# CYF2000127/MolNexTR

Hardware: AMD Instinct MI355X
Metric: molecules/sec (384x384, bs32 per GPU), full predict hot path (higher is better)
Workload: dtype fp16x3

## Files before the change

### molnextr_amd/csrc/engine.hip

```cpp
#include "../../include/molnextr_hip.h"

#include <hip/hip_runtime.h>

#include <time.h>
#include <cmath>
#include <cstdint>
#include <cstdio>
#include <cstring>
#include <map>
#include <memory>
#include <string>
#include <tuple>
#include <unordered_map>
#include <vector>

#include "dec_types.h"
#include "kernels.h"
#include "kvq.h"

using namespace mnx;

namespace {

thread_local std::string g_create_error;

struct W16 {
    void* p = nullptr;
    size_t lo = 0;
    float oscale = 1.f;
};
struct BlockW {
    float *ln1_g, *ln1_b, *table, *qkv_b, *proj_b, *ln2_g, *ln2_b, *fc1_b, *fc2_b;
    W16 qkv_w, proj_w, fc1_w, fc2_w;
};
struct StageW {
    std::vector<BlockW> blocks;
    float *m_g = nullptr, *m_b = nullptr;
    W16 m_w;
    int C = 0, heads = 0;
};
enum { SPL_QKV = 1, SPL_ATTN = 2, SPL_PROJ = 4, SPL_FC1 = 8, SPL_FC2 = 16, SPL_MERGE = 32, SPL_ALL = 63 };
struct GraphKey {
    int slots, rows, trace, forced, tile;
    bool operator<(const GraphKey& o) const {
        return std::tie(slots, rows, trace, forced, tile) < std::tie(o.slots, o.rows, o.trace, o.forced, o.tile);
    }
};

}

#ifndef MNX_PLANE_SKEW
#define MNX_PLANE_SKEW 4352
#endif
static constexpr size_t PLANE_SKEW = MNX_PLANE_SKEW;

struct mnx_engine {
    mnx_config cfg;
    int device = 0;
    std::string err;
    std::vector<void*> allocs;
    size_t bytes = 0;
    float *pe_wt = nullptr, *pe_b = nullptr, *pe_g = nullptr, *pe_beta = nullptr, *fn_g = nullptr, *fn_b = nullptr;
    std::vector<StageW> stages;
    float *xa = nullptr, *xb = nullptr;
    void *xn16 = nullptr, *qkv16 = nullptr, *attn16 = nullptr, *h16 = nullptr;
    size_t xn_lo = 0, qkv_lo = 0, attn_lo = 0, h_lo = 0;
    int dt = 0;
    int split_mask = SPL_ALL;
    int two_mask[4] = {0, 0, 0, 0};
    int two_first[4] = {0, 0, 0, 0}, two_last[4] = {1 << 30, 1 << 30, 1 << 30, 1 << 30};
    int* enc_flag = nullptr;
    float* zero_bias = nullptr;
    int zero_bias_n = 0;
    int tap_item = -1;
    float* tap_dst = nullptr;
    DecWeights dw{};
    DecBuffers db{};
    float* out_trace = nullptr;
    int* forced_ids = nullptr;
    BeamBuffers beam{};
    int* prep_bbox = nullptr;
    int* prep_bbox_batch = nullptr;
    float* beam_hidden = nullptr;
    int* host_flag = nullptr;
    std::map<GraphKey, hipGraphExec_t> graphs;
    hipStream_t enc_stream = nullptr;
    float* feat_ring[2] = {nullptr, nullptr};
    hipEvent_t ev_enc_done[2] = {nullptr, nullptr}, ev_feat_free[2] = {nullptr, nullptr}, ev_poll[2] = {nullptr, nullptr};
    int* slot_lists = nullptr;
    int* rowc_seq = nullptr;
    TokenClasses* tc_dev = nullptr;
    bool have_tc = false;
    int n_chunk_bufs = 0;
    bool use_graph = true;
    int dec_tile = -1, dec_tile_ff = 4, dec_fused_max = 128;
    int dec_mid_max = 0;
    hipStream_t own_stream = nullptr;
    bool profiling = false;
    int prof_stride = 1;
    int prof_calls = 0;
    int prof_groups = 0;
    int prof_max_groups = 4;
    struct Ev { hipEvent_t a, b; double work; int kind; };
    std::vector<Ev> ev_pool;
    size_t ev_used = 0;
};

namespace {

#define HIPCHK(h, expr)                                                                                   \
    do {                                                                                                  \
        hipError_t e_ = (expr);                                                                           \
        if (e_ != hipSuccess) {                                                                           \
            (h)->err = std::string(#expr) + ": " + hipGetErrorString(e_);                                 \
            return MNX_ERR_HIP;                                                                           \
        }                                                                                                 \
    } while (0)

#define MNXCHK(expr)                                                                                      \
    do {                                                                                                  \
        const int rc_ = (expr);                                                                           \
        if (rc_ != MNX_OK) return rc_;                                                                    \
    } while (0)

struct Packer {
    mnx_engine* h;
    std::unordered_map<std::string, const mnx_weight_desc*> by_name;
    std::vector<std::string> problems;
    float* staging = nullptr;
    size_t staging_elems = 0;

    const mnx_weight_desc* find(const std::string& name, std::initializer_list<int64_t> shape) {
        auto it = by_name.find(name);
        if (it == by_name.end()) {
            problems.push_back("missing " + name);
            return nullptr;
        }
        const mnx_weight_desc* d = it->second;
        bool ok = d->ndim == (int)shape.size() && d->data != nullptr;
        int i = 0;
        for (int64_t s : shape) ok = ok && d->shape[i++] == s;
        if (!ok) {
            std::string got = "[";
            for (int k = 0; k < d->ndim; ++k) got += std::to_string(d->shape[k]) + (k + 1 < d->ndim ? "," : "");
            problems.push_back("shape " + name + ": got " + got + "]");
            return nullptr;
        }
        return d;
    }
    void* dalloc(size_t bytes) {
        void* p = nullptr;
        if (hipMalloc(&p, bytes ? bytes : 16) != hipSuccess) {
            problems.push_back("hipMalloc failed for " + std::to_string(bytes) + " bytes");
            return nullptr;
        }
        h->allocs.push_back(p);
        h->bytes += bytes;
        return p;
    }
    float* up32(const float* host, size_t n) {
        float* p = (float*)dalloc(n * sizeof(float));
        if (p && hipMemcpy(p, host, n * sizeof(float), hipMemcpyHostToDevice) != hipSuccess)
            problems.push_back("hipMemcpy H2D failed");
        return p;
    }
    float* f32(const std::string& name, std::initializer_list<int64_t> shape) {
        const mnx_weight_desc* d = find(name, shape);
        if (!d) return nullptr;
        size_t n = 1;
// ... 494 lines not shown
    h->err = "encoder features are not finite (an activation left the fp16 range of compute_dtype FP16 / FP16X3, or the "
             "input holds NaN / Inf): use MNX_DTYPE_BF16X3 or MNX_DTYPE_FP32 for this checkpoint";
    return MNX_ERR_RANGE;
}

static int encode_impl(mnx_engine* h, const char* name, const void* images, int fmt, int32_t B, float* features_out,
                       void* stream) {
    if (!h) return MNX_ERR_INVALID_ARG;
    if (!images || !features_out || B < 1) { h->err = std::string(name) + ": null/empty argument"; return MNX_ERR_INVALID_ARG; }
    if (fmt == MNX_IMG_GRAY8 && ((uintptr_t)images & 3)) { h->err = std::string(name) + ": gray must be 4-byte aligned"; return MNX_ERR_INVALID_ARG; }
    if (B > h->cfg.max_batch) { h->err = std::string(name) + ": B exceeds max_batch"; return MNX_ERR_CAPACITY; }
    hipStream_t s = (hipStream_t)stream;
    const mnx_config& c = h->cfg;
    const int dt = h->dt;
    HIPCHK(h, hipSetDevice(h->device));
    int Hh = c.img_size / c.patch, Ww = Hh, C = c.embed_dim;
    float* cur = h->xa;
    float* other = h->xb;
    int item = 0;
    auto tap = [&](size_t elems) -> hipError_t {
        hipError_t e = hipSuccess;
        if (h->tap_item == item && h->tap_dst)
            e = hipMemcpyAsync(h->tap_dst, cur, elems * sizeof(float), hipMemcpyDeviceToDevice, s);
        ++item;
        return e;
    };
    const bool bracket = h->profiling && (h->prof_calls++ % h->prof_stride) == 0 && h->prof_groups < h->prof_max_groups;
    if (bracket) ++h->prof_groups;
    auto timed = [&](int kind, double work, auto&& launch) -> hipError_t {
        if (!bracket) return launch();
        if (h->ev_used == h->ev_pool.size()) {
            mnx_engine::Ev ev{};
            hipError_t e1 = hipEventCreate(&ev.a), e2 = hipEventCreate(&ev.b);
            if (e1 != hipSuccess || e2 != hipSuccess) return e1 != hipSuccess ? e1 : e2;
            h->ev_pool.push_back(ev);
        }
        mnx_engine::Ev& ev = h->ev_pool[h->ev_used++];
        ev.work = work; ev.kind = kind;
        hipError_t e0 = hipEventRecord(ev.a, s);
        if (e0 != hipSuccess) return e0;
        e0 = launch();
        if (e0 != hipSuccess) return e0;
        return hipEventRecord(ev.b, s);
    };
    const double es = (double)dt_size(dt);
    const bool split = dt_split(dt);
    int stage_now = 0, block_now = 0;
    auto terms_of = [&](int cls) {
        if (!(h->split_mask & cls)) return 1;
        const bool in_range = block_now >= h->two_first[stage_now] && block_now <= h->two_last[stage_now];
        return (in_range && (h->two_mask[stage_now] & cls)) ? 2 : 3;
    };
    auto planes_for = [&](int consumer_cls) { return split && terms_of(consumer_cls) == 2 ? 1 : 2; };
    auto gemm = [&](int epi, const void* A, size_t a_lo, const W16& Wt, void* Cc, size_t c_lo, const float* bias,
                    const float* resid, int M, int N, int K, int cls, int c_planes = 2) -> hipError_t {
        SplitArgs sp;
        sp.a_lo = a_lo; sp.w_lo = Wt.lo; sp.c_lo = c_lo; sp.oscale = Wt.oscale;
        sp.terms = terms_of(cls);
        sp.c_planes = c_planes;
        return timed((cls != SPL_MERGE && std::min(N, K) >= 512) ? 4 : 0, 2.0 * (double)M * (double)N * (double)K,
                     [&]() { return launch_gemm16(dt, epi, A, Wt.p, Cc, bias, resid, M, N, K, s, split ? &sp : nullptr); });
    };
    auto ln = [&](const float* x, const float* g, const float* b, void* y16, float* y32, int M, int Cc, int planes = 2) -> hipError_t {
        return timed(1, (double)M * Cc * (4.0 + (y16 ? es * planes / 2 : 0.0) + (y32 ? 4.0 : 0.0)),
                     [&]() { return launch_layernorm16(dt, x, g, b, y16, y32, M, Cc, 1e-5f, s, h->xn_lo, y32 ? h->enc_flag : nullptr, planes); });
    };
    if (fmt == MNX_IMG_GRAY8)
        HIPCHK(h, timed(3, (double)B * ((double)c.img_size * c.img_size + (double)Hh * Ww * C * 4.0), [&]() {
            return launch_patch_embed_gray8((const uint8_t*)images, h->pe_wt, h->pe_b, h->pe_g, h->pe_beta, cur, B, c.img_size, C, s);
        }));
    else
        HIPCHK(h, timed(3, (double)B * (3.0 * c.img_size * c.img_size + (double)Hh * Ww * C) * 4.0, [&]() {
            return launch_patch_embed((const float*)images, h->pe_wt, h->pe_b, h->pe_g, h->pe_beta, cur, B, c.img_size, C, s);
        }));
    HIPCHK(h, tap((size_t)B * Hh * Ww * C));
    for (int si = 0; si < c.n_stages; ++si) {
        StageW& st = h->stages[si];
        stage_now = si;
        const int M = B * Hh * Ww;
        for (size_t bi = 0; bi < st.blocks.size(); ++bi) {
            const BlockW& w = st.blocks[bi];
            block_now = (int)bi;
            const int shift = (bi % 2 == 0) ? 0 : c.window / 2;
            HIPCHK(h, ln(cur, w.ln1_g, w.ln1_b, h->xn16, nullptr, M, C, planes_for(SPL_QKV)));
            HIPCHK(h, gemm(EPI_BIAS_16, h->xn16, h->xn_lo, w.qkv_w, h->qkv16, h->qkv_lo, w.qkv_b, nullptr, M, 3 * C, C, SPL_QKV));
            HIPCHK(h, timed(2, (double)M * C * 4.0 * es, [&]() {
                return launch_window_attn(dt, h->qkv16, w.table, h->attn16, B, Hh, Ww, C, st.heads, shift, s, h->qkv_lo,
                                          h->attn_lo, (h->split_mask & SPL_ATTN) ? 3 : 1);
            }));
            HIPCHK(h, gemm(EPI_RESID_F32, h->attn16, h->attn_lo, w.proj_w, cur, 0, w.proj_b, cur, M, C, C, SPL_PROJ));
            HIPCHK(h, ln(cur, w.ln2_g, w.ln2_b, h->xn16, nullptr, M, C, planes_for(SPL_FC1)));
            HIPCHK(h, gemm(EPI_GELU_16, h->xn16, h->xn_lo, w.fc1_w, h->h16, h->h_lo, w.fc1_b, nullptr, M, 4 * C, C, SPL_FC1, planes_for(SPL_FC2)));
            HIPCHK(h, gemm(EPI_RESID_F32, h->h16, h->h_lo, w.fc2_w, cur, 0, w.fc2_b, cur, M, C, 4 * C, SPL_FC2));
            HIPCHK(h, tap((size_t)M * C));
        }
        if (si + 1 < c.n_stages) {
            block_now = (int)st.blocks.size() - 1;
            HIPCHK(h, launch_merge_ln16(dt, cur, st.m_g, st.m_b, h->xn16, B, Hh, Ww, C, 1e-5f, s, h->xn_lo, planes_for(SPL_MERGE)));
            HIPCHK(h, gemm(EPI_BIAS_F32, h->xn16, h->xn_lo, st.m_w, other, 0, h->zero_bias, nullptr, M / 4, 2 * C, 4 * C, SPL_MERGE));
            std::swap(cur, other);
            Hh /= 2; Ww /= 2; C *= 2;
            HIPCHK(h, tap((size_t)B * Hh * Ww * C));
        }
    }
    HIPCHK(h, ln(cur, h->fn_g, h->fn_b, nullptr, features_out, B * Hh * Ww, C));
    return MNX_OK;
}

int mnx_encode(mnx_engine* h, const float* images, int32_t B, float* features_out, void* stream) {
    return encode_impl(h, "mnx_encode", images, MNX_IMG_F32, B, features_out, stream);
}

int mnx_encode_gray8(mnx_engine* h, const uint8_t* gray, int32_t B, float* features_out, void* stream) {
    return encode_impl(h, "mnx_encode_gray8", gray, MNX_IMG_GRAY8, B, features_out, stream);
}

}

namespace {

int caller_stream(mnx_engine* h, void* stream, hipStream_t* s) {
    HIPCHK(h, hipSetDevice(h->device));
    *s = (hipStream_t)stream;
    if (!*s) {
        if (!h->own_stream) HIPCHK(h, hipStreamCreate(&h->own_stream));
        *s = h->own_stream;
    }
    return MNX_OK;
}

template <typename T>
int lazy_alloc(mnx_engine* h, T** p, size_t bytes) {
    if (*p) return MNX_OK;
    HIPCHK(h, hipMalloc((void**)p, bytes));
    h->allocs.push_back(*p);
    h->bytes += bytes;
    return MNX_OK;
}

int project_memory(mnx_engine* h, const float* feats, int n, int blk0, hipStream_t s) {
    const mnx_config& c = h->cfg;
    const int S = h->db.S, D = c.dec_dim;
    char* memkv = h->db.mem_kv + (size_t)blk0 * c.dec_layers * 2 * c.dec_heads * kvq_block_bytes(h->db.Sq);
    HIPCHK(h, launch_sgemm_tn(feats, h->dw.w_enc, h->dw.b_enc, h->db.memory, n * S, D, h->dw.enc_dim, s));
    HIPCHK(h, launch_sgemm_tn(h->db.memory, h->dw.w_memkv, h->dw.b_memkv, h->db.mem_kv32, n * S, c.dec_layers * 2 * D, D, s, S));
    HIPCHK(h, kvq_pack_enqueue(h->db.mem_kv32, memkv, n * c.dec_layers * 2 * c.dec_heads, S, h->db.Sq, s));
    return MNX_OK;
}

struct FeatRing {
    mnx_engine* h;
    const void* images;
    int fmt;
    int n_img, ref_batch, n_chunks, grp;
    int first[2] = {-1, -1}, count[2] = {0, 0};
    bool used[2] = {false, false};
    int next_enc = 0;

    int refill() {
        const size_t img_bytes = (size_t)h->cfg.img_size * h->cfg.img_size * (fmt == MNX_IMG_GRAY8 ? 1 : 3 * sizeof(float));
        for (int i = 0; i < 2; ++i) {
            if (first[i] >= 0 || next_enc >= n_chunks) continue;
            const int cnt = std::min(grp, n_chunks - next_enc);
            const int f = next_enc * ref_batch, n = std::min(cnt * ref_batch, n_img - f);
            if (used[i]) HIPCHK(h, hipStreamWaitEvent(h->enc_stream, h->ev_feat_free[i], 0));
            MNXCHK(encode_impl(h, fmt == MNX_IMG_GRAY8 ? "mnx_encode_gray8" : "mnx_encode", (const char*)images + (size_t)f * img_bytes,
                               fmt, n, h->feat_ring[i], h->enc_stream));
            HIPCHK(h, hipEventRecord(h->ev_enc_done[i], h->enc_stream));
            first[i] = next_enc;
            count[i] = cnt;
            next_enc += cnt;
        }
        return MNX_OK;
    }
    int find(int k) const {
        for (int i = 0; i < 2; ++i)
            if (first[i] >= 0 && k >= first[i] && k < first[i] + count[i]) return i;
        return -1;
    }
    int end(int i) const { return first[i] + count[i]; }
    const float* feats(int i, int k) const {
        return h->feat_ring[i] + (size_t)(k - first[i]) * ref_batch * h->db.S * h->dw.enc_dim;
    }
    int release(int i, hipStream_t s) {
        HIPCHK(h, hipEventRecord(h->ev_feat_free[i], s));
        used[i] = true;
        first[i] = -1;
        return MNX_OK;
    }
};

struct DrainGuard {
    mnx_engine* h;
    hipStream_t s;
    ~DrainGuard() { (void)hipStreamSynchronize(h->enc_stream); (void)hipStreamSynchronize(s); }
};

int tick_tile(const mnx_engine* h, int rows) {
    const mnx_config& c = h->cfg;
    if (c.dec_ff != 1024 || c.dec_heads != 8 || c.dec_dim != 256 || c.max_len + 1 > 512 || h->db.S > 160) return 0;
    if (h->dec_tile == 0 || rows % 16 || rows > h->db.fpart_rows) return 0;
    if (rows > h->dec_fused_max) {
        if (rows > h->dec_mid_max) return 0;
        return 2000 + 100 * 4 + 16;
    }
    const int r = h->dec_tile > 0 ? h->dec_tile : (rows <= 64 ? 2 : 4);
    return 100 * r + h->dec_tile_ff;
}

hipError_t enqueue_tick(mnx_engine* h, int slots, int rows, float* trace, int trace_rows, hipStream_t s, const int* forced) {
    return dec_enqueue_tick(h->dw, h->db, slots, rows, trace, trace_rows, s, nullptr, forced, tick_tile(h, rows));
}

template <typename F>
int capture_graph(mnx_engine* h, const char* what, hipStream_t s, F&& enqueue, hipGraphExec_t* out) {
    *out = nullptr;
    HIPCHK(h, hipStreamBeginCapture(s, hipStreamCaptureModeThreadLocal));
    hipGraph_t g = nullptr;
    hipError_t e = enqueue();
    const hipError_t e2 = hipStreamEndCapture(s, &g);
    if (e == hipSuccess) e = e2;
    const char* step = "capture";
    if (e == hipSuccess) {
        step = "instantiate";
        e = hipGraphInstantiate(out, g, nullptr, nullptr, 0);
    }
    if (g) hipGraphDestroy(g);
    if (e != hipSuccess) {
        *out = nullptr;
        h->err = std::string(what) + " " + step + " failed: " + hipGetErrorString(e);
        return MNX_ERR_HIP;
    }
    return MNX_OK;
}

int get_tick_graph(mnx_engine* h, int slots, int rows, float* trace, int trace_rows, hipStream_t s, hipGraphExec_t* out,
                   const int* forced = nullptr) {
    *out = nullptr;
    if (!h->use_graph) return MNX_OK;
    const GraphKey key{slots, rows, trace ? trace_rows : 0, forced ? trace_rows : 0, tick_tile(h, rows)};
    auto it = h->graphs.find(key);
    if (it != h->graphs.end()) { *out = it->second; return MNX_OK; }
    MNXCHK(capture_graph(h, "decode tick", s, [&]() { return enqueue_tick(h, slots, rows, trace, trace_rows, s, forced); }, out));
    h->graphs[key] = *out;
    return MNX_OK;
}

template <typename F>
int run_steps(mnx_engine* h, hipGraphExec_t exec, F&& enqueue, int slots, int max_len, hipStream_t s) {
    for (int t = 0; t < max_len; t += 8) {
        for (int i = 0; i < std::min(8, max_len - t); ++i) HIPCHK(h, exec ? hipGraphLaunch(exec, s) : enqueue());
        HIPCHK(h, dec_enqueue_status(h->db, slots, s));
        HIPCHK(h, hipMemcpyAsync(h->host_flag, &h->db.st->n_active, sizeof(int), hipMemcpyDeviceToHost, s));
        HIPCHK(h, hipStreamSynchronize(s));
        if (*h->host_flag == 0) break;
    }
    return MNX_OK;
}

int decode_greedy_impl(mnx_engine* h, const float* features, int32_t B, const int32_t* chunk_id, int32_t max_len,
                       int32_t stop_on_eos, const int32_t* forced_ids, int32_t* tokens, int32_t* lengths, float* token_logp,
                       float* hidden, float* logits_trace, void* stream) {
    if (!h) return MNX_ERR_INVALID_ARG;
    if (!features || !tokens || !lengths || B < 1) { h->err = "mnx_decode_greedy: null/empty argument"; return MNX_ERR_INVALID_ARG; }
    if (B > ROW_TILE || max_len < 1 || max_len > h->cfg.max_len) {
        h->err = "mnx_decode_greedy: B must be <= 32 and max_len <= cfg.max_len";
        return MNX_ERR_CAPACITY;
    }
    const mnx_config& c = h->cfg;
    hipStream_t s;
    MNXCHK(caller_stream(h, stream, &s));
    MNXCHK(project_memory(h, features, B, 0, s));
    HIPCHK(h, dec_enqueue_reset(h->db, s));
    HIPCHK(h, dec_enqueue_admit_rows(h->db, chunk_id, B, max_len, stop_on_eos, s));
    float* trace = nullptr;
    if (logits_trace) {
        MNXCHK(lazy_alloc(h, &h->out_trace, (size_t)c.max_len * ROW_TILE * c.vocab * 4));
        trace = h->out_trace;
    }
    const int* forced = nullptr;
    if (forced_ids) {
        MNXCHK(lazy_alloc(h, &h->forced_ids, (size_t)ROW_TILE * c.max_len * 4));
        HIPCHK(h, hipMemcpy2DAsync(h->forced_ids, (size_t)h->db.T * 4, forced_ids, (size_t)max_len * 4, (size_t)max_len * 4, B,
                                   hipMemcpyDeviceToDevice, s));
        forced = h->forced_ids;
    }
    hipGraphExec_t exec = nullptr;
    MNXCHK(get_tick_graph(h, ROW_TILE, ROW_TILE, trace, B, s, &exec, forced));
    MNXCHK(run_steps(h, exec, [&]() { return enqueue_tick(h, ROW_TILE, ROW_TILE, trace, B, s, forced); }, ROW_TILE, max_len, s));
    HIPCHK(h, gather_enqueue(h->db, nullptr, B, max_len, tokens, lengths, token_logp, hidden, s));
    if (logits_trace) HIPCHK(h, hipMemcpyAsync(logits_trace, trace, (size_t)max_len * B * c.vocab * 4, hipMemcpyDeviceToDevice, s));
    HIPCHK(h, hipStreamSynchronize(s));
    return MNX_OK;
}

int decode_beam_groups(mnx_engine* h, const float* const* feats, int G, int ref_batch, int n_total, int beam, int n_best,
                       int max_len, int32_t* tokens, int32_t* lengths, float* scores, float* hidden, hipStream_t s) {
    const int D = h->cfg.dec_dim, T = h->db.T, B = n_total;
    BeamBuffers& bm = h->beam;
    constexpr int POOL = ROW_TILE * MAX_BEAM;
    const int pool_stride = std::min(MAX_BEAM, POOL / B);
    if (pool_stride < n_best) { h->err = "beam search: n_best x images exceeds the hypothesis pool (256)"; return MNX_ERR_CAPACITY; }
    MNXCHK(lazy_alloc(h, &bm.bs, sizeof(BeamState)));
    MNXCHK(lazy_alloc(h, &bm.blp, (size_t)MAX_BEAM_IMGS * MAX_BEAM * BEAM_LP_STRIDE * 4));
    MNXCHK(lazy_alloc(h, &bm.anc, (size_t)MAX_BEAM_IMGS * MAX_BEAM * (T + 1) * 4));
    MNXCHK(lazy_alloc(h, &bm.ptok, (size_t)POOL * T * 4));
    if (hidden) MNXCHK(lazy_alloc(h, &bm.phid, (size_t)POOL * T * D * 4));
    bm.B = B; bm.K = beam; bm.n_best = n_best; bm.anc_stride = T + 1; bm.ref_batch = ref_batch; bm.pool_stride = pool_stride;
    BeamBuffers run = bm;
    if (!hidden) run.phid = nullptr;
    for (int g = 0; g < G; ++g)
        MNXCHK(project_memory(h, feats[g], std::min(ref_batch, B - g * ref_batch), g * ref_batch, s));
    HIPCHK(h, dec_enqueue_reset(h->db, s));
    HIPCHK(h, beam_enqueue_init(h->db, run, max_len, s));
    const int rows = (B * beam + ROW_TILE - 1) / ROW_TILE * ROW_TILE;
    auto step = [&]() { return dec_enqueue_tick(h->dw, h->db, rows, rows, nullptr, 0, s, &run); };
    hipGraphExec_t exec = nullptr;
    if (h->use_graph) MNXCHK(capture_graph(h, "beam step", s, step, &exec));
    struct ExecGuard {
        hipGraphExec_t e;
        ~ExecGuard() { if (e) hipGraphExecDestroy(e); }
    } guard{exec};
    MNXCHK(run_steps(h, exec, step, rows, max_len, s));
    HIPCHK(h, beam_enqueue_gather(h->db, run, max_len, tokens, lengths, scores, hidden, s));
    HIPCHK(h, hipStreamSynchronize(s));
    return MNX_OK;
}

}

extern "C" {

int mnx_decode_greedy(mnx_engine* h, const float* features, int32_t B, const int32_t* chunk_id, int32_t max_len,
                      int32_t stop_on_eos, int32_t* tokens, int32_t* lengths, float* token_logp, float* hidden,
                      float* logits_trace, void* stream) {
    return decode_greedy_impl(h, features, B, chunk_id, max_len, stop_on_eos, nullptr, tokens, lengths, token_logp, hidden,
                              logits_trace, stream);
}

int mnx_decode_forced(mnx_engine* h, const float* features, int32_t B, const int32_t* chunk_id, int32_t max_len,
                      const int32_t* forced_ids, int32_t* argmax_ids, int32_t* lengths, float* forced_logp,
                      float* logits_trace, void* stream) {
    if (h && !forced_ids) { h->err = "mnx_decode_forced: forced_ids is null"; return MNX_ERR_INVALID_ARG; }
    return decode_greedy_impl(h, features, B, chunk_id, max_len, 1, forced_ids, argmax_ids, lengths, forced_logp, nullptr,
                              logits_trace, stream);
}

int mnx_decode_beam(mnx_engine* h, const float* features, int32_t B, int32_t beam, int32_t n_best, int32_t max_len,
                    int32_t* tokens, int32_t* lengths, float* scores, float* hidden, void* stream) {
    if (!h) return MNX_ERR_INVALID_ARG;
    if (!features || !tokens || !lengths || !scores || B < 1) {
        h->err = "mnx_decode_beam: null/empty argument";
        return MNX_ERR_INVALID_ARG;
    }
    const mnx_config& c = h->cfg;
    if (B > ROW_TILE || beam < 1 || beam > MAX_BEAM || n_best < 1 || n_best > beam || max_len < 1 ||
        max_len > c.max_len || c.max_len + 1 > BEAM_ANC_MAX || c.vocab > BEAM_LP_STRIDE || B * beam > h->db.slots) {
        h->err = "mnx_decode_beam: B <= 32, 1 <= n_best <= beam <= 8, max_len <= cfg.max_len (<= 511), B x beam <= dec_slots required";
        return MNX_ERR_CAPACITY;
    }
    hipStream_t s;
    MNXCHK(caller_stream(h, stream, &s));
    return decode_beam_groups(h, &features, 1, B, B, beam, n_best, max_len, tokens, lengths, scores, hidden, s);
}

int mnx_predict_beam(mnx_engine* h, const float* images, int32_t n_img, int32_t ref_batch, int32_t beam, int32_t max_len,
                     int32_t* tokens, int32_t* lengths, float* scores, int32_t* n_atoms, int32_t* atom_idx,
                     uint8_t* edges, int32_t kmax, void* stream) {
    if (!h) return MNX_ERR_INVALID_ARG;
    if (!images || !tokens || !lengths || !scores || !n_atoms || !atom_idx || !edges || n_img < 1) {
        h->err = "mnx_predict_beam: null/empty argument";
        return MNX_ERR_INVALID_ARG;
    }
    if (!h->have_tc) { h->err = "mnx_predict_beam: call mnx_set_token_classes first"; return MNX_ERR_INVALID_ARG; }
    const mnx_config& c = h->cfg;
    if (ref_batch < 1 || ref_batch > ROW_TILE || ref_batch > c.max_batch || beam < 1 || beam > MAX_BEAM || max_len < 1 ||
        max_len > c.max_len || kmax < 1 || kmax > h->db.kmax || c.max_len + 1 > BEAM_ANC_MAX || c.vocab > BEAM_LP_STRIDE ||
        ref_batch * beam > h->db.slots) {
        h->err = "mnx_predict_beam: ref_batch <= min(32, max_batch), beam <= 8, max_len <= cfg.max_len (<= 511), kmax <= cfg.max_atoms, "
                 "ref_batch x beam <= dec_slots required";
        return MNX_ERR_CAPACITY;
    }
    hipStream_t s;
    MNXCHK(caller_stream(h, stream, &s));
    const int D = c.dec_dim;
    int g_max = 8;
    if (const char* e = getenv("MNX_BEAM_GROUPS")) g_max = std::max(1, atoi(e));
    g_max = std::max(1, std::min({g_max, MAX_BEAM_IMGS / ref_batch, h->db.slots / (ref_batch * beam), h->db.mem_blocks / ref_batch}));
    MNXCHK(lazy_alloc(h, &h->beam_hidden, (size_t)MAX_BEAM_IMGS * c.max_len * D * 4));
    DrainGuard drain{h, s};
    HIPCHK(h, hipMemsetAsync(h->enc_flag, 0, sizeof(int), s));
    HIPCHK(h, hipEventRecord(h->ev_poll[0], s));
    HIPCHK(h, hipStreamWaitEvent(h->enc_stream, h->ev_poll[0], 0));
    const int n_chunks = (n_img + ref_batch - 1) / ref_batch;
    FeatRing ring{h, images, MNX_IMG_F32, n_img, ref_batch, n_chunks, std::max(1, c.max_batch / ref_batch)};
    for (int ck = 0; ck < n_chunks;) {
        MNXCHK(ring.refill());
        const int fb = ring.find(ck);
        if (fb < 0) { h->err = "mnx_predict_beam: internal: reference batch without features"; return MNX_ERR_HIP; }
        const int G = std::min(g_max, ring.end(fb) - ck);
        const int first = ck * ref_batch, n = std::min(G * ref_batch, n_img - first);
        HIPCHK(h, hipStreamWaitEvent(s, h->ev_enc_done[fb], 0));
        const float* feats[MAX_BEAM_IMGS];
        for (int g = 0; g < G; ++g) feats[g] = ring.feats(fb, ck + g);
        int32_t* tok = tokens + (size_t)first * max_len;
        MNXCHK(decode_beam_groups(h, feats, G, ref_batch, n, beam, 1, max_len, tok, lengths + first, scores + first, h->beam_hidden, s));
        ck += G;
        if (ck == ring.end(fb)) MNXCHK(ring.release(fb, s));
        int32_t* aidx = atom_idx + (size_t)first * kmax;
        HIPCHK(h, atoms_enqueue_raw(h->tc_dev, tok, lengths + first, n, max_len, kmax, aidx, n_atoms + first, s));
        for (int o = 0; o < n; o += ROW_TILE) {
            const int nb = std::min(ROW_TILE, n - o);
            HIPCHK(h, edges_enqueue(h->dw, h->db, h->beam_hidden + (size_t)o * max_len * D, nullptr, aidx + (size_t)o * kmax,
                                    n_atoms + first + o, nb, kmax, max_len, edges + (size_t)(first + o) * kmax * kmax, nullptr, s));
        }
    }
    HIPCHK(h, hipStreamSynchronize(s));
    return check_encoder_range(h, s);
}

int mnx_preprocess(mnx_engine* h, const uint8_t* rgb, int32_t height, int32_t width, int32_t pad,
                   int32_t pad_to_square, int32_t* crop_out, float* out, void* stream) {
    if (!h) return MNX_ERR_INVALID_ARG;
    if (!rgb || !out || height < 1 || width < 1 || pad < 0) { h->err = "mnx_preprocess: null/empty argument"; return MNX_ERR_INVALID_ARG; }
    if (height > 16384 || width > 16384 || pad > 4096) { h->err = "mnx_preprocess: image larger than 16384x16384"; return MNX_ERR_CAPACITY; }
    HIPCHK(h, hipSetDevice(h->device));
    HIPCHK(h, launch_preprocess(rgb, height, width, pad, pad_to_square ? 1 : 0, h->cfg.img_size, h->prep_bbox, crop_out, out,
                                (hipStream_t)stream));
    return MNX_OK;
}

int mnx_preprocess_batch(mnx_engine* h, const uint8_t* arena, const mnx_page* pages, int32_t n, int32_t max_height,
                         int32_t pad, int32_t pad_to_square, int32_t* crops_out, void* out, int32_t out_format,
                         void* stream) {
    if (!h) return MNX_ERR_INVALID_ARG;
    if (!arena || !pages || !out || n < 1) { h->err = "mnx_preprocess_batch: null/empty argument"; return MNX_ERR_INVALID_ARG; }
    if (out_format != MNX_IMG_F32 && out_format != MNX_IMG_GRAY8) {
        h->err = "mnx_preprocess_batch: out_format must be MNX_IMG_F32 or MNX_IMG_GRAY8";
        return MNX_ERR_INVALID_ARG;
    }
    if (max_height < 1 || max_height > 16384 || pad < 0 || pad > 4096) {
        h->err = "mnx_preprocess_batch: 1 <= max_height <= 16384 and 0 <= pad <= 4096 required";
        return MNX_ERR_INVALID_ARG;
    }
    if (((uintptr_t)arena & 15) || ((uintptr_t)pages & 7) || ((uintptr_t)out & 3) || ((uintptr_t)crops_out & 3)) {
        h->err = "mnx_preprocess_batch: arena must be 16-byte, pages 8-byte, out and crops_out 4-byte aligned";
        return MNX_ERR_INVALID_ARG;
    }
    if (n > MNX_PREP_MAX_PAGES) {
        h->err = "mnx_preprocess_batch: n " + std::to_string(n) + " exceeds MNX_PREP_MAX_PAGES = " + std::to_string(MNX_PREP_MAX_PAGES);
        return MNX_ERR_CAPACITY;
    }
    HIPCHK(h, hipSetDevice(h->device));
    HIPCHK(h, launch_preprocess_batch(arena, pages, n, max_height, pad, pad_to_square ? 1 : 0, h->cfg.img_size,
                                      h->prep_bbox_batch, crops_out, out, out_format == MNX_IMG_GRAY8, (hipStream_t)stream));
    return MNX_OK;
}

int mnx_edges(mnx_engine* h, const float* hidden, const int32_t* atom_idx, const int32_t* n_atoms, int32_t B,
              int32_t kmax, int32_t max_len, uint8_t* edges, double* scores, void* stream) {
    if (!h) return MNX_ERR_INVALID_ARG;
    if (!hidden || !atom_idx || !n_atoms || !edges || B < 1 || kmax < 1 || max_len < 1) {
        h->err = "mnx_edges: null/empty argument";
        return MNX_ERR_INVALID_ARG;
    }
    if (B > ROW_TILE || kmax > h->db.kmax) { h->err = "mnx_edges: B <= 32 and kmax <= cfg.max_atoms required"; return MNX_ERR_CAPACITY; }
    HIPCHK(h, hipSetDevice(h->device));
    HIPCHK(h, edges_enqueue(h->dw, h->db, hidden, nullptr, atom_idx, n_atoms, B, kmax, max_len, edges, scores, (hipStream_t)stream));
    return MNX_OK;
}

int mnx_set_token_classes(mnx_engine* h, const uint8_t* flags, int32_t n, int32_t lbracket, int32_t rbracket,
                          int32_t id_C, int32_t id_l, int32_t id_B, int32_t id_r) {
    if (!h || !flags || n < 1 || n > 256) return MNX_ERR_INVALID_ARG;
    HIPCHK(h, hipSetDevice(h->device));
    TokenClasses tc{};
    memcpy(tc.flags, flags, (size_t)n);
    tc.lbracket = lbracket; tc.rbracket = rbracket; tc.id_C = id_C; tc.id_l = id_l; tc.id_B = id_B; tc.id_r = id_r;
    tc.x0 = h->cfg.sym_offset; tc.y0 = h->cfg.sym_offset + h->cfg.coord_bins; tc.vocab = h->cfg.vocab;
    HIPCHK(h, hipMemcpy(h->tc_dev, &tc, sizeof(tc), hipMemcpyHostToDevice));
    h->have_tc = true;
    return MNX_OK;
}

int mnx_atom_scan(mnx_engine* h, const int32_t* tokens, const int32_t* lengths, int32_t n, int32_t T, int32_t kmax,
                  int32_t* atom_idx, int32_t* n_atoms, void* stream) {
    if (!h || !tokens || !lengths || !atom_idx || !n_atoms || n < 1 || T < 1 || kmax < 1) return MNX_ERR_INVALID_ARG;
    if (!h->have_tc) { h->err = "mnx_atom_scan: call mnx_set_token_classes first"; return MNX_ERR_INVALID_ARG; }
    HIPCHK(h, hipSetDevice(h->device));
    HIPCHK(h, atoms_enqueue_raw(h->tc_dev, tokens, lengths, n, T, kmax, atom_idx, n_atoms, (hipStream_t)stream));
    return MNX_OK;
}

int mnx_confidence(mnx_engine* h, const int32_t* tokens, const int32_t* lengths, const float* token_logp, int32_t n,
                   int32_t T, const int32_t* atom_idx, const int32_t* n_atoms, const double* edge_scores, int32_t kmax,
                   double* atom_scores, double* overall_score, void* stream) {
    if (!h) return MNX_ERR_INVALID_ARG;
    if (!tokens || !lengths || !token_logp || !atom_idx || !n_atoms || !edge_scores || !atom_scores || !overall_score ||
        n < 1 || T < 1 || kmax < 1) {
        h->err = "mnx_confidence: null/empty argument";
        return MNX_ERR_INVALID_ARG;
    }
    if (!h->have_tc) { h->err = "mnx_confidence: call mnx_set_token_classes first"; return MNX_ERR_INVALID_ARG; }
    if (T > 512 || kmax > h->db.kmax) { h->err = "mnx_confidence: T <= 512 and kmax <= cfg.max_atoms required"; return MNX_ERR_CAPACITY; }
    HIPCHK(h, hipSetDevice(h->device));
    HIPCHK(h, confidence_enqueue_raw(h->tc_dev, tokens, lengths, token_logp, n, T, kmax, atom_idx, n_atoms, edge_scores,
                                     atom_scores, overall_score, (hipStream_t)stream));
    return MNX_OK;
}

}

namespace {
struct ConfOut {
    float* token_logp;
    double *edge_scores, *atom_scores, *overall;
};
}

static int predict_impl(mnx_engine* h, const char* name, const void* images, int img_fmt, int32_t n_img, int32_t ref_batch,
                        int32_t max_len, int32_t stop_on_eos, int32_t* tokens, int32_t* lengths, int32_t* n_atoms,
                        int32_t* atom_idx, uint8_t* edges, int32_t kmax, const ConfOut* conf, void* stream) {
    if (!h) return MNX_ERR_INVALID_ARG;
    if (!images || !tokens || !lengths || !n_atoms || !atom_idx || !edges || n_img < 1 ||
        (conf && (!conf->edge_scores || !conf->atom_scores || !conf->overall))) {
        h->err = std::string(name) + ": null/empty argument";
        return MNX_ERR_INVALID_ARG;
    }
    if (img_fmt == MNX_IMG_GRAY8 && ((uintptr_t)images & 3)) { h->err = std::string(name) + ": gray must be 4-byte aligned"; return MNX_ERR_INVALID_ARG; }
    if (!h->have_tc) { h->err = std::string(name) + ": call mnx_set_token_classes first"; return MNX_ERR_INVALID_ARG; }
    const mnx_config& c = h->cfg;
    const int SL = h->db.slots;
    {
        const char* hit = ref_batch > MAX_REF_BATCH ? "MAX_REF_BATCH" : ref_batch > c.max_batch ? "cfg.max_batch"
                        : ref_batch > SL ? "cfg.dec_slots" : ref_batch > c.pe_len ? "cfg.pe_len" : nullptr;
        const int lim = ref_batch > MAX_REF_BATCH ? MAX_REF_BATCH : ref_batch > c.max_batch ? c.max_batch
                      : ref_batch > SL ? SL : c.pe_len;
        if (hit) {
            h->err = std::string(name) + ": ref_batch " + std::to_string(ref_batch) + " exceeds " + hit + " = " +
                     std::to_string(lim);
            return MNX_ERR_CAPACITY;
        }
    }
    if (ref_batch < 1 || max_len < 1 || max_len > c.max_len || kmax < 1 || kmax > h->db.kmax) {
        h->err = std::string(name) + ": 1 <= ref_batch, max_len <= cfg.max_len, kmax <= cfg.max_atoms required";
        return MNX_ERR_CAPACITY;
    }
    hipStream_t s;
    MNXCHK(caller_stream(h, stream, &s));
    const int n_chunks = (n_img + ref_batch - 1) / ref_batch;
    struct Chunk { int first, n, tag, admit_seq; std::vector<int> tiles; };
    std::vector<Chunk> live;
    std::vector<int> free_tiles;
    for (int i = h->n_chunk_bufs - 1; i >= 0; --i) free_tiles.push_back(i);
    int* pinned = h->host_flag;
    int* pin_slots = h->host_flag + 2 * (1 + MAX_CHUNKS);
    int bound = 0;
    std::vector<std::pair<int, int>> admits;
    HIPCHK(h, dec_enqueue_reset(h->db, s));
    HIPCHK(h, hipMemsetAsync(h->enc_flag, 0, sizeof(int), s));
    HIPCHK(h, hipEventRecord(h->ev_poll[0], s));
    HIPCHK(h, hipStreamWaitEvent(h->enc_stream, h->ev_poll[0], 0));
    int next = 0, done = 0, seq = 0;
    const char* trace_path = getenv("MNX_TRACE");
    FILE* tf = trace_path ? fopen(trace_path, "a") : nullptr;
    const std::unique_ptr<FILE, int (*)(FILE*)> tf_close(tf, fclose);
    DrainGuard drain{h, s};
    auto now_ms = []() { timespec ts; clock_gettime(CLOCK_MONOTONIC, &ts); return ts.tv_sec * 1e3 + ts.tv_nsec * 1e-6; };
    const double t_begin = now_ms();
    double host_wait_ms = 0.0;
    FeatRing ring{h, images, img_fmt, n_img, ref_batch, n_chunks, std::max(1, c.max_batch / ref_batch)};
    const int ticks_per_poll = 4;
    while (done < n_chunks) {
        MNXCHK(ring.refill());
        while (next < n_chunks) {
            const int fb = ring.find(next);
            if (fb < 0) break;
            const int first = next * ref_batch, n = std::min(ref_batch, n_img - first);
            const int n_tiles = (n + ROW_TILE - 1) / ROW_TILE;
            if ((int)free_tiles.size() < n_tiles) break;
            const bool idle = live.empty();
            hipError_t q = idle ? hipEventSynchronize(h->ev_enc_done[fb]) : hipEventQuery(h->ev_enc_done[fb]);
            if (q == hipErrorNotReady) break;
            if (q != hipSuccess) { h->err = std::string("encoder event: ") + hipGetErrorString(q); return MNX_ERR_HIP; }
            Chunk ck;
            ck.first = first; ck.n = n; ck.admit_seq = seq;
            for (int j = 0; j < n_tiles; ++j) { ck.tiles.push_back(free_tiles.back()); free_tiles.pop_back(); }
            ck.tag = ck.tiles[0];
            HIPCHK(h, hipStreamWaitEvent(s, h->ev_enc_done[fb], 0));
            for (int j = 0; j < n_tiles; ++j) {
                const float* feats = ring.feats(fb, next) + (size_t)j * ROW_TILE * h->db.S * h->dw.enc_dim;
                MNXCHK(project_memory(h, feats, std::min(ROW_TILE, n - j * ROW_TILE), ck.tiles[j] * ROW_TILE, s));
            }
            if (next + 1 == ring.end(fb)) MNXCHK(ring.release(fb, s));
            for (int j = 0; j < n_tiles; ++j) {
                const int tile = ck.tiles[j], nj = std::min(ROW_TILE, n - j * ROW_TILE);
                int* sl_dev = h->slot_lists + (size_t)tile * ROW_TILE;
                int* sl_pin = pin_slots + (size_t)tile * ROW_TILE;
                for (int i = 0; i < nj; ++i) sl_pin[i] = tile * ROW_TILE + i;
                HIPCHK(h, hipMemcpyAsync(sl_dev, sl_pin, (size_t)nj * 4, hipMemcpyHostToDevice, s));
                HIPCHK(h, dec_enqueue_admit(h->db, sl_dev, h->rowc_seq + j * ROW_TILE, nj, ck.tag, tile * ROW_TILE, max_len,
                                            stop_on_eos ? 1 : 0, s));
            }
            bound += n;
            admits.emplace_back(seq, n);
            live.push_back(std::move(ck));
            ++next;
        }
        if (live.empty()) continue;
        const int cap_step = bound <= 1024 ? 64 : bound <= 2048 ? 128 : 256;
        const int rows_cap = std::min(SL, (std::max(bound, 1) + cap_step - 1) / cap_step * cap_step);
        int hi_tile = 0;
        for (const Chunk& ck : live)
            for (int t : ck.tiles) hi_tile = std::max(hi_tile, t);
        const int scan = std::min(SL, std::max(((hi_tile + 1) * ROW_TILE + 1023) / 1024 * 1024, rows_cap));
        hipGraphExec_t exec = nullptr;
        MNXCHK(get_tick_graph(h, scan, rows_cap, nullptr, 0, s, &exec));
        for (int i = 0; i < ticks_per_poll; ++i)
            HIPCHK(h, exec ? hipGraphLaunch(exec, s) : enqueue_tick(h, scan, rows_cap, nullptr, 0, s, nullptr));
        HIPCHK(h, dec_enqueue_status(h->db, scan, s));
        int* snap = pinned + (seq & 1) * (1 + MAX_CHUNKS);
        HIPCHK(h, hipMemcpyAsync(snap, &h->db.st->n_active, (size_t)(1 + MAX_CHUNKS) * 4, hipMemcpyDeviceToHost, s));
        HIPCHK(h, hipEventRecord(h->ev_poll[seq & 1], s));
        if (seq > 0) {
            const int ps = seq - 1;
            const double tw0 = tf ? now_ms() : 0.0;
            HIPCHK(h, hipEventSynchronize(h->ev_poll[ps & 1]));
            if (tf) host_wait_ms += now_ms() - tw0;
            const int* sn = pinned + (ps & 1) * (1 + MAX_CHUNKS);
            {
                int after = 0;
                for (auto& a : admits) if (a.first > ps) after += a.second;
                bound = std::min(bound, sn[0] + after);
                while (!admits.empty() && admits.front().first <= ps) admits.erase(admits.begin());
            }
            for (size_t i = 0; i < live.size();) {
                Chunk& ck = live[i];
                if (ck.admit_seq <= ps && sn[1 + ck.tag] == 0) {
                    for (int j = 0; j < (int)ck.tiles.size(); ++j) {
                        const int o = ck.first + j * ROW_TILE, nj = std::min(ROW_TILE, ck.n - j * ROW_TILE);
                        int* sl_dev = h->slot_lists + (size_t)ck.tiles[j] * ROW_TILE;
                        int* o_idx = atom_idx + (size_t)o * kmax;
                        int* o_na = n_atoms + o;
                        float* o_logp = conf && conf->token_logp ? conf->token_logp + (size_t)o * max_len : nullptr;
                        double* o_scores = conf ? conf->edge_scores + (size_t)o * kmax * kmax : nullptr;
                        HIPCHK(h, gather_enqueue(h->db, sl_dev, nj, max_len, tokens + (size_t)o * max_len, lengths + o, o_logp,
                                                 nullptr, s));
                        HIPCHK(h, atoms_enqueue(h->db, h->tc_dev, sl_dev, nj, kmax, o_idx, o_na, s));
                        HIPCHK(h, edges_enqueue(h->dw, h->db, h->db.hidden, sl_dev, o_idx, o_na, nj, kmax, h->db.T,
                                                edges + (size_t)o * kmax * kmax, o_scores, s));
                        if (conf)
                            HIPCHK(h, confidence_enqueue(h->db, h->tc_dev, sl_dev, nj, kmax, o_idx, o_na, o_scores,
                                                         conf->atom_scores + (size_t)o * kmax, conf->overall + o, s));
                    }
                    for (int t : ck.tiles) free_tiles.push_back(t);
                    live.erase(live.begin() + i);
                    ++done;
                } else {
                    ++i;
                }
            }
        }
        if (tf) fprintf(tf, "%.3f seq %d live %zu next %d next_enc %d done %d free_tiles %zu\n", now_ms() - t_begin, seq,
                        live.size(), next, ring.next_enc, done, free_tiles.size());
        ++seq;
        if (seq > 200000) { h->err = std::string(name) + ": watchdog (decode did not terminate)"; return MNX_ERR_HIP; }
    }
    HIPCHK(h, hipStreamSynchronize(s));
    if (tf) fprintf(tf, "%.3f end host_wait_ms %.3f\n", now_ms() - t_begin, host_wait_ms);
    return check_encoder_range(h, s);
}

extern "C" {

int mnx_predict(mnx_engine* h, const float* images, int32_t n_img, int32_t ref_batch, int32_t max_len,
                int32_t stop_on_eos, int32_t* tokens, int32_t* lengths, int32_t* n_atoms, int32_t* atom_idx,
                uint8_t* edges, int32_t kmax, void* stream) {
    return predict_impl(h, "mnx_predict", images, MNX_IMG_F32, n_img, ref_batch, max_len, stop_on_eos, tokens, lengths, n_atoms, atom_idx,
                        edges, kmax, nullptr, stream);
}

int mnx_predict_confidence(mnx_engine* h, const float* images, int32_t n_img, int32_t ref_batch, int32_t max_len,
                           int32_t* tokens, int32_t* lengths, int32_t* n_atoms, int32_t* atom_idx, uint8_t* edges,
                           int32_t kmax, float* token_logp, double* edge_scores, double* atom_scores, double* overall_score,
                           void* stream) {
    const ConfOut conf{token_logp, edge_scores, atom_scores, overall_score};
    return predict_impl(h, "mnx_predict_confidence", images, MNX_IMG_F32, n_img, ref_batch, max_len, 1, tokens, lengths, n_atoms,
                        atom_idx, edges, kmax, &conf, stream);
}

int mnx_predict_gray8(mnx_engine* h, const uint8_t* gray, int32_t n_img, int32_t ref_batch, int32_t max_len,
                      int32_t* tokens, int32_t* lengths, int32_t* n_atoms, int32_t* atom_idx, uint8_t* edges, int32_t kmax,
                      float* token_logp, double* edge_scores, double* atom_scores, double* overall_score, void* stream) {
    if (!h) return MNX_ERR_INVALID_ARG;
    const int n_conf = !!token_logp + !!edge_scores + !!atom_scores + !!overall_score;
    if (n_conf != 0 && n_conf != 4) {
        h->err = "mnx_predict_gray8: the four confidence pointers must be all NULL or all set";
        return MNX_ERR_INVALID_ARG;
    }
    const ConfOut conf{token_logp, edge_scores, atom_scores, overall_score};
    return predict_impl(h, "mnx_predict_gray8", gray, MNX_IMG_GRAY8, n_img, ref_batch, max_len, 1, tokens, lengths, n_atoms,
                        atom_idx, edges, kmax, n_conf ? &conf : nullptr, stream);
}

int mnx_gemm_clock(mnx_engine* h, int32_t reset, double* mhz) {
    if (!h || !mhz) return MNX_ERR_INVALID_ARG;
    HIPCHK(h, hipSetDevice(h->device));
    HIPCHK(h, hipDeviceSynchronize());
    HIPCHK(h, x3_clock_read(mhz, reset != 0));
    return MNX_OK;
}

int mnx_probe_mfma(mnx_engine* h, int32_t ms_target, double* tflops, double* mhz, void* stream) {
    if (!h || !tflops || !mhz || ms_target < 1 || ms_target > 2000) return MNX_ERR_INVALID_ARG;
    HIPCHK(h, hipSetDevice(h->device));
    const int iters = (int)((double)ms_target * 1e-3 * 1.9e9 / 256.0);
    HIPCHK(h, mfma_probe(iters, (hipStream_t)stream, tflops, mhz));
    return MNX_OK;
}

int mnx_profile_enable(mnx_engine* h, int32_t enable) {
    if (!h) return MNX_ERR_INVALID_ARG;
    h->profiling = enable != 0;
    h->prof_stride = enable > 1 ? enable : 1;
// ... 154 lines not shown
```

Measured before the change: 2186.

## Ramp encoder group sizes to shorten pipeline fill and drain

Replaces the fixed encoder group size in the feature ring with a per-group plan. For the greedy decode path it starts with small groups that double up to the max and ends with two small tail groups. The aim is for decoding to start sooner and for less time to sit idle waiting on a large final encode. The cost is more encode launches at smaller batch sizes, which run less efficiently. The beam path keeps uniform groups.

```diff
diff --git a/molnextr_amd/csrc/engine.hip b/molnextr_amd/csrc/engine.hip
--- a/molnextr_amd/csrc/engine.hip
+++ b/molnextr_amd/csrc/engine.hip
@@ -15,6 +15,7 @@
 #include <vector>
 
 #include "dec_types.h"
+#include "group_plan.h"
 #include "kernels.h"
 #include "kvq.h"
 
@@ -815,16 +816,18 @@
     mnx_engine* h;
     const void* images;
     int fmt;
-    int n_img, ref_batch, n_chunks, grp;
+    int n_img, ref_batch, n_chunks;
+    std::vector<int> plan;
     int first[2] = {-1, -1}, count[2] = {0, 0};
     bool used[2] = {false, false};
     int next_enc = 0;
+    size_t next_grp = 0;
 
     int refill() {
         const size_t img_bytes = (size_t)h->cfg.img_size * h->cfg.img_size * (fmt == MNX_IMG_GRAY8 ? 1 : 3 * sizeof(float));
         for (int i = 0; i < 2; ++i) {
-            if (first[i] >= 0 || next_enc >= n_chunks) continue;
-            const int cnt = std::min(grp, n_chunks - next_enc);
+            if (first[i] >= 0 || next_grp >= plan.size()) continue;
+            const int cnt = plan[next_grp++];
             const int f = next_enc * ref_batch, n = std::min(cnt * ref_batch, n_img - f);
             if (used[i]) HIPCHK(h, hipStreamWaitEvent(h->enc_stream, h->ev_feat_free[i], 0));
             MNXCHK(encode_impl(h, fmt == MNX_IMG_GRAY8 ? "mnx_encode_gray8" : "mnx_encode", (const char*)images + (size_t)f * img_bytes,
@@ -1056,7 +1059,7 @@
     HIPCHK(h, hipEventRecord(h->ev_poll[0], s));
     HIPCHK(h, hipStreamWaitEvent(h->enc_stream, h->ev_poll[0], 0));
     const int n_chunks = (n_img + ref_batch - 1) / ref_batch;
-    FeatRing ring{h, images, MNX_IMG_F32, n_img, ref_batch, n_chunks, std::max(1, c.max_batch / ref_batch)};
+    FeatRing ring{h, images, MNX_IMG_F32, n_img, ref_batch, n_chunks, uniform_group_plan(n_chunks, c.max_batch / ref_batch)};
     for (int ck = 0; ck < n_chunks;) {
         MNXCHK(ring.refill());
         const int fb = ring.find(ck);
@@ -1232,7 +1235,12 @@
     auto now_ms = []() { timespec ts; clock_gettime(CLOCK_MONOTONIC, &ts); return ts.tv_sec * 1e3 + ts.tv_nsec * 1e-6; };
     const double t_begin = now_ms();
     double host_wait_ms = 0.0;
-    FeatRing ring{h, images, img_fmt, n_img, ref_batch, n_chunks, std::max(1, c.max_batch / ref_batch)};
+    FeatRing ring{h, images, img_fmt, n_img, ref_batch, n_chunks, encoder_group_plan(n_chunks, c.max_batch / ref_batch)};
+    if (tf) {
+        fprintf(tf, "plan n_chunks %d grp_max %d groups", n_chunks, std::max(1, c.max_batch / ref_batch));
+        for (int g : ring.plan) fprintf(tf, " %d", g);
+        fprintf(tf, "\n");
+    }
     const int ticks_per_poll = 4;
     while (done < n_chunks) {
         MNXCHK(ring.refill());
diff --git a/molnextr_amd/csrc/group_plan.h b/molnextr_amd/csrc/group_plan.h
--- /dev/null
+++ b/molnextr_amd/csrc/group_plan.h
@@ -0,0 +1,31 @@
+#pragma once
+#include <algorithm>
+#include <vector>
+
+namespace mnx {
+
+inline std::vector<int> uniform_group_plan(int n_chunks, int grp_max) {
+    grp_max = std::max(1, grp_max);
+    std::vector<int> plan;
+    for (int k = 0; k < n_chunks; k += grp_max) plan.push_back(std::min(grp_max, n_chunks - k));
+    return plan;
+}
+
+inline std::vector<int> encoder_group_plan(int n_chunks, int grp_max) {
+    grp_max = std::max(1, grp_max);
+    if (n_chunks <= grp_max) return n_chunks > 0 ? std::vector<int>{n_chunks} : std::vector<int>{};
+    const int u = std::max(1, grp_max / 8);
+    const int n_tail = 2;
+    std::vector<int> plan;
+    int left = n_chunks - n_tail * u;
+    for (int g = u, i = 0; left > 0 && g < grp_max; ++i, g = i < 2 ? u : g * 2) {
+        const int cnt = std::min(g, left);
+        plan.push_back(cnt);
+        left -= cnt;
+    }
+    for (; left > 0; left -= std::min(grp_max, left)) plan.push_back(std::min(grp_max, left));
+    for (int i = 0; i < n_tail; ++i) plan.push_back(u);
+    return plan;
+}
+
+}
```

New measurement: 2142. 0.98x the previous value.
